# MarioPasc/MGA-YOLO

Measured on AMD Instinct MI355X. Metric: images/s (MaskCBAM fwd+bwd step at P3/P4/P5, YOLOv8n 640x640), higher is better.
Workload: dtype f32; 1 GPU; YOLOv8n+MGA-CBAM P3/P4/P5, 32x640x640 synthetic per GPU, fp32 (BASELINE.json configs[1]); batch_per_gpu=32, global_batch=32, parallelism=dp1, launch=hipGraph replay, 1 graph/step, handoff_kernels=True

## Files before the change

mga_yolo_amd/csrc/api_bwd.hip:

```cpp
#include "host.cuh"
#include "bwd.cuh"
#include "nhwc_bwd.cuh"

static int backward_args(const mgacbam_bwd_level_t& L, NhwcBwdArgs& N, Sig& sig) {
  const bool nhwc = (L.flags & MGACBAM_LAYOUT_NHWC) != 0;
  if (!L.x || !L.gy || !L.ctx || !L.scratch || !L.gx) return fail(MGACBAM_E_NULL, "backward: x / gy / ctx / scratch / gx is NULL");
  if (!L.gw1 || !L.gb1 || !L.gw2 || !L.gb2 || !L.gwsa || !L.gbeta) return fail(MGACBAM_E_NULL, "backward: NULL parameter-gradient pointer");
  if (L.gmask && !L.mask) return fail(MGACBAM_E_NULL, "backward: gmask requested but mask is NULL");
  if (int e = check_level("backward", L)) return e;
  const int VEC = level_vec(nhwc, L.C, L.H, L.W, L.dtype);
  const size_t need = VEC * elem_size(L.dtype);
  if (!aligned_to(L.x, need) || !aligned_to(L.gy, need) || !aligned_to(L.gx, need) || !aligned_to(L.ctx, 16) ||
      !aligned_to(L.scratch, 16) || (L.gmask && !aligned_to(L.gmask, nhwc ? 4 : 16)) || (nhwc && L.mask && !aligned_to(L.mask, 4)))
    return fail(MGACBAM_E_ALIGN, "backward%s: x/gy/gx must be %zu-byte aligned, ctx/scratch 16-byte", nhwc ? " (NHWC)" : "", need);
  const ScratchLayout SL = scratch_layout(L.B, L.C, L.H, L.W, L.p.hidden, L.p.k, nhwc, VEC);
  if (int e = check_ctx_capacity("backward", L)) return e;
  if (int e = check_capacity("backward", "scratch", SL.total, L.scratch_bytes)) return e;
  BwdArgs& A = N.a;
  A.x = L.x; A.mask = L.mask; A.gy = L.gy; A.gx = L.gx; A.gmask = L.gmask;
  A.gw1 = L.gw1; A.gb1 = L.gb1; A.gw2 = L.gw2; A.gb2 = L.gb2; A.gwsa = L.gwsa; A.gbeta = L.gbeta;
  level_setup(L, A);
  A.s = scratch_ptrs(L.scratch, SL);
  A.nconv = A.g.B * conv_tiles(A.t, A.g.H, A.g.W);
  A.nwsa = A.g.B * wsa_tiles(A.t, A.g.H, A.g.W);
  A.npg = params_blocks(A.g);
  A.merged = 0;
  A.vec = VEC;
  sig = Sig{L.dtype, VEC, L.mask != nullptr, L.p.k, L.gmask != nullptr, 0};
  if (nhwc) {
    N.n = nhwc_geo(L.C, L.H, L.W, VEC);
    N.ncb = (L.C + kNhwcFoldC - 1) / kNhwcFoldC;
    A.nt = N.n.nchunk;
    A.ncg = N.ncb;
    A.bflag0 = A.cflag0 = A.mbflag0 = A.mcflag0 = A.wflag0 = A.sflag0 = 0;
    sig.nhwc = 1;
    sig.weight = L.C;
    return 0;
  }
  A.nt = chan_tiles(A.t, A.g.H, A.g.W, VEC);
  A.ncg = 0;
  const SyncLayout S = sync_layout(L.B, L.C, static_cast<size_t>(L.H) * L.W);
  A.bflag0 = static_cast<int>(S.bflag); A.cflag0 = static_cast<int>(S.cflag);
  A.mbflag0 = static_cast<int>(S.mbflag); A.mcflag0 = static_cast<int>(S.mcflag);
  A.wflag0 = static_cast<int>(S.wflag); A.sflag0 = static_cast<int>(S.sflag);
  sig.weight = L.C * A.t.chan_tx;
  sig.proj = (L.flags & MGACBAM_BWD_HAVE_PROJ) && L.gmask != nullptr;
  A.g.proj_h = (sig.proj && L.p.hidden <= MGACBAM_PROJ_MAX_HIDDEN) ? L.p.hidden : 0;
  return 0;
}

template <typename SmemOf>
static size_t group_smem(const Group<BwdArgs>& G, SmemOf smem_of) {
  size_t smem = 0;
  for (int l = 0; l < G.n; ++l) smem = std::max(smem, smem_of(G.lv[l]));
  return smem;
}
static size_t reduce2_smem(const Tune& t) { return (64 + static_cast<size_t>(std::max(kPghLds, kBlock / t.pool_tx))) * sizeof(float); }
static int launch_convT(Group<BwdArgs>& G, int k, hipStream_t st) {
  const size_t smem = group_smem(G, [&](const BwdArgs& a) { return convT_smem(a.t, k); });
  const int grid = fill_starts(G, G.lv, G.n, [](const BwdArgs& a) { return a.nconv; });
  switch (k) {
    case 3: LAUNCH(k_bwd_convT<3>, grid, smem, st, G); break;
    case 5: LAUNCH(k_bwd_convT<5>, grid, smem, st, G); break;
    case 7: LAUNCH(k_bwd_convT<7>, grid, smem, st, G); break;
    default: LAUNCH(k_bwd_convT<0>, grid, smem, st, G); break;
  }
  return launch_status("k_bwd_convT");
}
static int launch_wsa(Group<BwdArgs>& G, int k, hipStream_t st) {
  const size_t smem = group_smem(G, [&](const BwdArgs& a) { return wsa_smem(a.t, k); });
  const int grid = fill_starts(G, G.lv, G.n, [](const BwdArgs& a) { return a.nwsa; });
  switch (k) {
    case 3: LAUNCH(k_bwd_wsa<3>, grid, smem, st, G); break;
    case 5: LAUNCH(k_bwd_wsa<5>, grid, smem, st, G); break;
    case 7: LAUNCH(k_bwd_wsa<7>, grid, smem, st, G); break;
    default: LAUNCH(k_bwd_wsa<0>, grid, smem, st, G); break;
  }
  return launch_status("k_bwd_wsa");
}
static int launch_params(Group<BwdArgs>& G, hipStream_t st) {
  const size_t smem = group_smem(G, [](const BwdArgs& a) { return params_smem(a.g); });
  const int grid = fill_starts(G, G.lv, G.n, [](const BwdArgs& a) { return a.npg; });
  LAUNCH(k_bwd_params, grid, smem, st, G);
  return launch_status("k_bwd_params");
}

static int backward_group(BwdArgs* lv, int n, const Sig& sig, int stages, hipStream_t st) {
  Group<BwdArgs> G;
  G.n = n;
  constexpr int kReduce2MaxCpt = 4;
  const int cpt = group_cpt(lv, n, kReduce2MaxCpt);
  for (int l = 0; l < n; ++l) {
    lv[l].t.pool_cpt = cpt;
    const int cpb = (kBlock / lv[l].t.pool_tx) * cpt;
    lv[l].ncg = (lv[l].g.C + cpb - 1) / cpb;
    G.lv[l] = lv[l];
  }

  bool fold = (stages & MGACBAM_BWD_FOLD) && (stages & MGACBAM_BWD_REDUCE1) && (stages & MGACBAM_BWD_CONVT);
  for (int l = 0; l < n && fold; ++l) {
    const int TP = lv[l].t.chan_tx * sig.vec;
    fold = TP >= kSyncPx && TP >= lv[l].g.W && 8 * (((lv[l].t.conv_th + lv[l].g.k) * lv[l].g.W + TP - 1) / TP + 1) <= 512 &&
           lv[l].nconv <= lv[l].g.B * lv[l].nflag;
  }
  const bool fuse = (stages & MGACBAM_BWD_FUSE) != 0;
  bool merge = fold && fuse && (stages & MGACBAM_BWD_REDUCE2) && (stages & MGACBAM_BWD_WSA) && sig.k == 7 && knobs().bwd_merge;
  for (int l = 0; l < n && merge; ++l) merge = lv[l].nwsa <= lv[l].g.B * lv[l].nflag && lv[l].ncg <= lv[l].g.C && lv[l].nconv % lv[l].g.B == 0;
  if (merge) {
    R12Group R;
    R.g.n = n;
    size_t smem = 0;
    for (int l = 0; l < n; ++l) {
      lv[l].merged = 1; lv[l].bflag0 = lv[l].mbflag0; lv[l].cflag0 = lv[l].mcflag0;
      R.g.lv[l] = lv[l];
      smem = std::max({smem, reduce1_smem(lv[l].g, sig.vec), convT_smem(lv[l].t, sig.k), wsa_smem(lv[l].t, sig.k),
                       reduce2_smem(lv[l].t)});
    }
    int tot = 0;
    for (int p = 0; p < 4; ++p) {
      for (int l = 0; l < n; ++l) {
        R.seg[p][l] = tot;
        tot += p == 0 ? xcd_grid(lv[l].g.B, lv[l].nt) : p == 1 ? pad8(lv[l].nconv) : p == 2 ? pad8(lv[l].nwsa) : sweep_blocks(lv[l], lv[l].t.pool_tx, cpt);
      }
      R.seg[p][n] = tot;
    }
    const int grid = tot;
#define CALL_R12B(CPTV) LAUNCH((k_bwd_r12<TT, VV, CPTV>), grid, smem, st, R)
#define CALL_R12(Tt, Vv) { using TT = Tt; constexpr int VV = Vv; DISPATCH_CPT(cpt, CALL_R12B); }
    DISPATCH_T_VEC(sig.dtype, sig.vec, CALL_R12);
#undef CALL_R12
#undef CALL_R12B
    if (int e = launch_status("k_bwd_r12")) return e;
    for (int l = 0; l < n; ++l) G.lv[l] = lv[l];
  }
  if (fold && !merge) {
    size_t smem = 0;
    for (int l = 0; l < n; ++l) smem = std::max({smem, reduce1_smem(lv[l].g, sig.vec), convT_smem(lv[l].t, sig.k)});
    const int grid = fill_starts(G, lv, n, [&](const BwdArgs& a) { return xcd_grid(a.g.B, a.nt) + pad8(a.nconv); });
#define CALL_R1F(Tt, Vv) if (sig.k == 7) LAUNCH((k_bwd_reduce1_fold<Tt, Vv, 7>), grid, smem, st, G); else LAUNCH((k_bwd_reduce1_fold<Tt, Vv, 0>), grid, smem, st, G)
    DISPATCH_T_VEC(sig.dtype, sig.vec, CALL_R1F);
#undef CALL_R1F
    if (int e = launch_status("k_bwd_reduce1_fold")) return e;
  }
  if ((stages & MGACBAM_BWD_REDUCE1) && !fold) {
    size_t smem = 0;
    for (int l = 0; l < n; ++l) smem = std::max(smem, reduce1_smem(lv[l].g, sig.vec));
    const int grid = fill_starts(G, lv, n, [&](const BwdArgs& a) { return xcd_grid(a.g.B, a.nt); });
#define CALL_R1(Tt, Vv) LAUNCH((k_bwd_reduce1<Tt, Vv>), grid, smem, st, G)
    DISPATCH_T_VEC(sig.dtype, sig.vec, CALL_R1);
#undef CALL_R1
    if (int e = launch_status("k_bwd_reduce1")) return e;
  }
  if ((stages & MGACBAM_BWD_CONVT) && !fold)
    if (int e = launch_convT(G, sig.k, st)) return e;
  const bool fuse_pg = fuse && (stages & MGACBAM_BWD_APPLY) && (stages & MGACBAM_BWD_PARAMGRAD);
  const bool fuse_wsa = fuse && (stages & MGACBAM_BWD_REDUCE2) && (stages & MGACBAM_BWD_WSA) && sig.k == 7;
  if ((stages & MGACBAM_BWD_REDUCE2) && !merge) {
    size_t smem = 0;
    for (int l = 0; l < n; ++l) {
      smem = std::max(smem, reduce2_smem(lv[l].t));
      if (fuse_wsa) smem = std::max(smem, wsa_smem(lv[l].t, sig.k));
    }
    const int grid = fill_starts(G, lv, n, [&](const BwdArgs& a) { return (fuse_wsa ? pad8(a.nwsa) : 0) + sweep_blocks(a, a.t.pool_tx, cpt); });
#define CALL_R22(CPTV) if (fuse_wsa) LAUNCH((k_bwd_reduce2<TT, VV, CPTV, true>), grid, smem, st, G); else LAUNCH((k_bwd_reduce2<TT, VV, CPTV, false>), grid, smem, st, G)
#define CALL_R2(Tt, Vv) { using TT = Tt; constexpr int VV = Vv; DISPATCH_CPT(cpt, CALL_R22); }
    DISPATCH_T_VEC(sig.dtype, sig.vec, CALL_R2);
#undef CALL_R2
#undef CALL_R22
    if (int e = launch_status("k_bwd_reduce2")) return e;
  }
  if ((stages & MGACBAM_BWD_WSA) && !fuse_wsa && !merge)
    if (int e = launch_wsa(G, sig.k, st)) return e;
  if ((stages & MGACBAM_BWD_PARAMGRAD) && !fuse_pg)
    if (int e = launch_params(G, st)) return e;
  if (stages & MGACBAM_BWD_APPLY) {
    size_t smem = 0;
    for (int l = 0; l < n; ++l) {
      smem = std::max(smem, bwd_apply_smem(lv[l].g, sig.vec));
      if (fuse_pg) smem = std::max(smem, params_smem(lv[l].g));
    }
    const int grid = fill_starts(G, lv, n, [&](const BwdArgs& a) { return (fuse_pg ? pad8(a.npg) : 0) + xcd_grid(a.g.B, a.nt); });
#define CALL_AP2(GM) if (fuse_pg) LAUNCH((k_bwd_apply<TT, VV, GM, true>), grid, smem, st, G); else LAUNCH((k_bwd_apply<TT, VV, GM, false>), grid, smem, st, G)
#define CALL_AP(Tt, Vv) { using TT = Tt; constexpr int VV = Vv; if (sig.gmask) { CALL_AP2(true); } else { CALL_AP2(false); } }
    DISPATCH_T_VEC(sig.dtype, sig.vec, CALL_AP);
#undef CALL_AP
#undef CALL_AP2
    if (int e = launch_status("k_bwd_apply")) return e;
  }
  return 0;
}

static int backward_group_nhwc(NhwcBwdArgs* lv, int n, const Sig& sig, int stages, hipStream_t st) {
  Group<NhwcBwdArgs> G;
  Group<BwdArgs> GB;
  G.n = GB.n = n;
  for (int l = 0; l < n; ++l) { G.lv[l] = lv[l]; GB.lv[l] = lv[l].a; }
  auto chunks = [&]() { return fill_starts(G, lv, n, [&](const NhwcBwdArgs& a) { return xcd_grid(a.a.g.B, a.n.nchunk); }); };
  if (stages & MGACBAM_BWD_REDUCE1) {
    size_t smem = 0;
    for (int l = 0; l < n; ++l) smem = std::max(smem, nhwc_reduce1_smem(lv[l].a.g, sig.vec));
    const int grid = chunks();
#define CALL_NR1(Tt, Vv) LAUNCH((k_bwd_reduce1_nhwc<Tt, Vv>), grid, smem, st, G)
    DISPATCH_T_VEC8(sig.dtype, sig.vec, CALL_NR1);
#undef CALL_NR1
    if (int e = launch_status("k_bwd_reduce1_nhwc")) return e;
  }
  if (stages & MGACBAM_BWD_CONVT)
    if (int e = launch_convT(GB, sig.k, st)) return e;
  if (stages & MGACBAM_BWD_REDUCE2) {
    size_t smem = 0;
    for (int l = 0; l < n; ++l) smem = std::max(smem, nhwc_reduce2_smem(lv[l].a.g));
    const int grid = chunks();
#define CALL_NR2(Tt, Vv) LAUNCH((k_bwd_reduce2_nhwc<Tt, Vv>), grid, smem, st, G)
    DISPATCH_T_VEC8(sig.dtype, sig.vec, CALL_NR2);
#undef CALL_NR2
    if (int e = launch_status("k_bwd_reduce2_nhwc")) return e;
    const int fgrid = fill_starts(G, lv, n, [&](const NhwcBwdArgs& a) { return a.a.g.B * a.ncb; });
    LAUNCH(k_bwd_fold_nhwc, fgrid, 0, st, G);
    if (int e = launch_status("k_bwd_fold_nhwc")) return e;
  }
  if (stages & MGACBAM_BWD_WSA)
    if (int e = launch_wsa(GB, sig.k, st)) return e;
  if (stages & MGACBAM_BWD_PARAMGRAD)
    if (int e = launch_params(GB, st)) return e;
  if (stages & MGACBAM_BWD_APPLY) {
    size_t smem = 0;
    for (int l = 0; l < n; ++l) smem = std::max(smem, nhwc_bwd_apply_smem(lv[l].a.g));
    const int grid = fill_starts(G, lv, n, [&](const NhwcBwdArgs& a) { return xcd_grid(a.a.g.B, a.n.ntile); });
#define CALL_NAP(Tt, Vv) if (sig.gmask) LAUNCH((k_bwd_apply_nhwc<Tt, Vv, true>), grid, smem, st, G); else LAUNCH((k_bwd_apply_nhwc<Tt, Vv, false>), grid, smem, st, G)
    DISPATCH_T_VEC8(sig.dtype, sig.vec, CALL_NAP);
#undef CALL_NAP
// ... 30 lines not shown
```

mga_yolo_amd/csrc/args.cuh:

```cuda
#pragma once
#include <stddef.h>
#include <stdint.h>

namespace mgacbam {

struct Geo {
  int B, C, H, W, HW;
  int hidden, k;
  int use_sigmoid;
  float thr, eps;
  int proj_h;
};
constexpr int kProjMax = 4;
constexpr int kGateR = 16;
constexpr int kSyncPx = 16;

struct CtxPtrs {
  float* S; float* use; float* den;
  float* avg; float* mx; float* mavg;
  int* valid; int* amax;
  float* h_avg; float* h_mx; float* ca;
  float* planes; int* cidx; float* sa;
  float* proj;
  int* sync;
};

struct ParamPtrs { const float* w1; const float* b1; const float* w2; const float* b2; const float* wsa; const float* beta; };

struct Tune {
  int pool_tx;
  int pool_cpt;
  int chan_tx;
  int conv_twq;
  int conv_th;
  int wsa_th;
  int apply_rows;
  int gate_rows;
  int gate_tx;
  int gate_span;
};

struct FwdArgs {
  const void* x; const float* mask; void* y;
  CtxPtrs c; ParamPtrs p; Geo g; Tune t;
  int nflag;
  int fused;
  unsigned spin_limit;
  int fault;
  long long* trace;
};

struct ScratchPtrs {
  float* A_part;
  float* gpre;
  float* gplanes;
  float* gwsa_part;
  float* gz;
  float* gbq;
  float* gh_avg;
  float* gh_mx;
  float* pgh;
};

struct BwdArgs {
  const void* x; const float* mask; const void* gy; void* gx; float* gmask;
  float* gw1; float* gb1; float* gw2; float* gb2; float* gwsa; float* gbeta;
  CtxPtrs c; ParamPtrs p; ScratchPtrs s; Geo g; Tune t;
  int nt;
  int nconv;
  int nwsa;
  int npg;
  int ncg;
  int nflag;
  int bflag0;
  int cflag0;
  int wflag0;
  int sflag0;
  int mbflag0, mcflag0;
  int merged;
  unsigned spin_limit;
  int vec;
  long long* trace;
};

struct NhwcGeo {
  int cs, lcs;
  int ng;
  int ch;
  int ntile;
  int rp;
  int nchunk;
};
constexpr int kNhwcMaxChunks = 64;
constexpr int kNhwcFoldC = 64;

static inline size_t align16(size_t v) { return (v + 15) & ~size_t(15); }

constexpr int kGroupMax = 4;
template <typename Args>
struct Group {
  int n;
  int start[kGroupMax + 1];
  Args lv[kGroupMax];
};

}
```

mga_yolo_amd/csrc/bwd.cuh:

```cuda
#pragma once
#include "args.cuh"
#include "common.cuh"
#include "tile.cuh"

namespace mgacbam {

constexpr int kPghLds = 2048;

template <typename T, int VEC, bool FOLD = false>
__device__ __forceinline__ void bwd_reduce1_body(const BwdArgs& A, const int bid, float* smem) {
  const Geo& g = A.g;
  const int tid = threadIdx.x;
  const int TX = A.t.chan_tx, lt = ilog2(TX);
  const int tx = tid & (TX - 1), ty = tid >> lt, TY = kBlock >> lt;
  const int nv = g.HW / VEC;
  const int ntile = A.nt;
  int b, tile;
  if (!xcd_sample_part(bid, g.B, ntile, b, tile)) return;
  const int i = tile * TX + tx;
  const bool active = i < nv;
  const int ii = active ? i : nv - 1;
  const size_t base = static_cast<size_t>(b) * g.C * g.HW + static_cast<size_t>(ii) * VEC;
  const T* xp = static_cast<const T*>(A.x) + base;
  const T* gp = static_cast<const T*>(A.gy) + base;
  const float a = softplusf_(*A.p.beta);
  float* s_ca = smem;
  float* s_aq = smem + g.C;
  float* sm = s_aq + 2 * g.C;
  for (int c = tid; c < g.C; c += kBlock) s_ca[c] = A.c.ca[static_cast<size_t>(b) * g.C + c];

  float sav[VEC];
  load_vec<float, VEC>(A.c.sa + static_cast<size_t>(b) * g.HW + static_cast<size_t>(ii) * VEC, sav);
  const float live = active ? 1.f : 0.f;
  float accp[VEC];
#pragma unroll
  for (int e = 0; e < VEC; ++e) accp[e] = 0.f;
  __syncthreads();

#pragma unroll 4
  for (int c = ty; c < g.C; c += TY) {
    float xv[VEC], gv[VEC];
    load_vec<T, VEC>(xp + static_cast<size_t>(c) * g.HW, xv);
    load_vec<T, VEC>(gp + static_cast<size_t>(c) * g.HW, gv);
    const float cac = s_ca[c];
    float pa = 0.f, pq = 0.f;
#pragma unroll
    for (int e = 0; e < VEC; ++e) {
      const float p = xv[e] * gv[e] * live;
      accp[e] += cac * p;
      pa += p * sav[e];
      pq += p * (cac * sav[e] - 1.f);
    }
    pa = wave_group_sum(pa, TX);
    pq = wave_group_sum(pq, TX);
    if (tx == 0) { s_aq[c] = pa; s_aq[g.C + c] = pq; }
  }
#pragma unroll
  for (int e = 0; e < VEC; ++e) sm[tid * VEC + e] = accp[e];
  __syncthreads();
  float* part = A.s.A_part + (static_cast<size_t>(b) * ntile + tile) * 2 * g.C;
  if (FOLD && A.merged) { for (int c = tid; c < 2 * g.C; c += kBlock) st_agent(part + c, s_aq[c]); }
  else { for (int c = tid; c < 2 * g.C; c += kBlock) part[c] = s_aq[c]; }
  if (ty == 0 && active) {
    for (int r = 1; r < TY; ++r) {
      const int o = (r * TX + tx) * VEC;
#pragma unroll
      for (int e = 0; e < VEC; ++e) accp[e] += sm[o + e];
    }
    float gpre[VEC];
#pragma unroll
    for (int e = 0; e < VEC; ++e) gpre[e] = a * accp[e] * sav[e] * (1.f - sav[e]);
    float* gq = A.s.gpre + static_cast<size_t>(b) * g.HW + static_cast<size_t>(i) * VEC;
    if (FOLD) {
#pragma unroll
      for (int e = 0; e < VEC; ++e) st_agent(gq + e, gpre[e]);
    } else {
      store_vec<float, VEC>(gq, gpre);
    }
  }
  if (FOLD) handoff_publish(A.c.sync + A.bflag0 + static_cast<size_t>(b) * A.nflag + tile);
}

template <typename T, int VEC>
__global__ __launch_bounds__(kBlock) void k_bwd_reduce1(const Group<BwdArgs> G) {
  extern __shared__ __align__(16) float smem[];
  int local;
  const int l = find_level(G, blockIdx.x, local);
  bwd_reduce1_body<T, VEC>(G.lv[l], local, smem);
}

template <int K, bool COH>
__device__ __forceinline__ void bwd_convT_body(const BwdArgs& A, const int local, float* smem) {
  const Geo& g = A.g;
  const int k = K ? K : g.k;
  const ConvTile c = conv_tile(g, A.t, k, local, A.t.conv_th);
  const int tid = threadIdx.x;
  float* wts = smem;
  float* tg = smem + ((3 * k * k + 3) & ~3);
  for (int i = tid; i < 3 * k * k; i += kBlock) wts[i] = A.p.wsa[i];
  const float* gpre = A.s.gpre + static_cast<size_t>(c.b) * g.HW;
  bool bad = false;
  if (COH) {
    int* own = A.c.sync + A.cflag0 + local;
    const int gen = static_cast<int>(static_cast<unsigned>(ld_agent(own)) + 1u);
    const int TP = A.t.chan_tx * A.vec;
    const int ra = max(c.y0 - c.pad, 0), rb = min(c.y0 + c.TH - 1 + c.pad, g.H - 1);
    bad = handoff_wait(A.c.sync + A.bflag0 + static_cast<size_t>(c.b) * A.nflag, (ra * g.W) / TP, ((rb + 1) * g.W - 1) / TP, gen,
                       A.c.sync + static_cast<size_t>(g.B) * A.nflag, A.spin_limit);
    if (tid == 0 && !A.merged) __hip_atomic_fetch_add(own, 1, __ATOMIC_RELAXED, __HIP_MEMORY_SCOPE_AGENT);
  }
  stage_window<8>(tg, 1, c.PH, c.PW, c.y0 - c.pad, c.x0 - c.pad, g, [&](int, int off) { return COH ? ld_agent(gpre + off) : gpre[off]; });
  __syncthreads();
  const int TWQ = A.t.conv_twq;
  const int py = tid / TWQ, q = tid - py * TWQ;
  constexpr int KK = K ? K : 1;
  const bool publish = COH && A.merged;
  if (py >= c.TH && !publish) return;
  float acc[3][4];
#pragma unroll
  for (int p = 0; p < 3; ++p)
#pragma unroll
    for (int e = 0; e < 4; ++e) acc[p][e] = 0.f;
  if (py >= c.TH) {
  } else if (K) {
#pragma unroll 1
    for (int i = 0; i < KK; ++i) {
      const float* row = tg + (py + i) * c.PW + q * 4;
      float r[4 + KK - 1];
#pragma unroll
      for (int t = 0; t < 4 + KK - 1; ++t) r[t] = row[t];
#pragma unroll
      for (int p = 0; p < 3; ++p) {
        const float* wr = wts + (p * KK + (KK - 1 - i)) * KK;
#pragma unroll
        for (int j = 0; j < KK; ++j) {
          const float wv = wr[KK - 1 - j];
#pragma unroll
          for (int e = 0; e < 4; ++e) acc[p][e] += wv * r[e + j];
        }
      }
    }
  } else {
    for (int i = 0; i < k; ++i) {
      const float* row = tg + (py + i) * c.PW + q * 4;
      for (int j = 0; j < k; ++j) {
#pragma unroll
        for (int p = 0; p < 3; ++p) {
          const float wv = wts[(p * k + (k - 1 - i)) * k + (k - 1 - j)];
#pragma unroll
          for (int e = 0; e < 4; ++e) acc[p][e] += wv * row[e + j];
        }
      }
    }
  }
  const int yg = c.y0 + py;
  if (py < c.TH && yg < g.H) {
#pragma unroll
    for (int e = 0; e < 4; ++e) {
      const int xg = c.x0 + q * 4 + e;
      if (xg < g.W) {
#pragma unroll
        for (int p = 0; p < 3; ++p) {
          float* dst = A.s.gplanes + (static_cast<size_t>(c.b) * 3 + p) * g.HW + yg * g.W + xg;
          const float v = bad ? __builtin_nanf("") : acc[p][e];
          if (publish) st_agent(dst, v); else *dst = v;
        }
      }
    }
  }
  if (publish) handoff_publish(A.c.sync + A.cflag0 + local);
}

template <int K>
__global__ __launch_bounds__(kBlock) void k_bwd_convT(const Group<BwdArgs> G) {
  extern __shared__ __align__(16) float smem[];
  int local;
  const int lvl = find_level(G, blockIdx.x, local);
  bwd_convT_body<K, false>(G.lv[lvl], local, smem);
}

template <typename T, int VEC, int K>
__global__ __launch_bounds__(kBlock) void k_bwd_reduce1_fold(const Group<BwdArgs> G) {
  extern __shared__ __align__(16) float smem[];
  int local;
  const int l = find_level(G, blockIdx.x, local);
  const BwdArgs& A = G.lv[l];
  const int tiles = ((A.g.B + 7) / 8) * 8 * A.nt;
  if (local >= tiles) {
    if (local - tiles < A.nconv) bwd_convT_body<K, true>(A, local - tiles, smem);
    return;
  }
  bwd_reduce1_body<T, VEC, true>(A, local, smem);
}

template <int K, bool COH = false>
__device__ __forceinline__ void bwd_wsa_body(const BwdArgs& A, const int local, float* smem) {
  const Geo& g = A.g;
  const int k = K ? K : g.k;
  const ConvTile c = conv_tile(g, A.t, k, local, A.t.wsa_th);
  const int tid = threadIdx.x;
  const int plane_elems = c.PH * c.PW;
  float* tg = smem;
  float* tp = tg + plane_elems;
  float* accs = tp + 3 * plane_elems;
  const float* gpre = A.s.gpre + static_cast<size_t>(c.b) * g.HW;
  const float* pl = A.c.planes + static_cast<size_t>(c.b) * 3 * g.HW;
  bool bad = false;
  if (COH) {
    int* own = A.c.sync + A.wflag0 + local;
    const int gen = static_cast<int>(static_cast<unsigned>(ld_agent(own)) + 1u);
    const int TP = A.t.chan_tx * A.vec;
    const int ra = max(c.y0 - c.pad, 0), rb = min(c.y0 + c.TH - 1 + c.pad, g.H - 1);
    bad = handoff_wait(A.c.sync + A.bflag0 + static_cast<size_t>(c.b) * A.nflag, (ra * g.W) / TP, ((rb + 1) * g.W - 1) / TP, gen,
                       A.c.sync + static_cast<size_t>(g.B) * A.nflag, A.spin_limit);
    if (tid == 0) __hip_atomic_fetch_add(own, 1, __ATOMIC_RELAXED, __HIP_MEMORY_SCOPE_AGENT);
  }
  stage_window<8>(tg, 4, c.PH, c.PW, c.y0 - c.pad, c.x0 - c.pad, g,
                   [&](int p, int off) { return p == 0 ? (COH ? ld_agent(gpre + off) : gpre[off]) : pl[static_cast<size_t>(p - 1) * g.HW + off]; });
  __syncthreads();
  constexpr int KK = K ? K : 1;
  const int nout = 3 * k * k;
  if (K) {
    const int nitems = 3 * KK * c.TH;
    for (int item = tid; item < nitems; item += kBlock) {
      const int pi = item / c.TH, r = item - pi * c.TH;
      const int p = pi / KK, i = pi - p * KK;
      const float* prow = tp + p * plane_elems + (r + i) * c.PW;
      const float* grow = tg + (r + c.pad) * c.PW + c.pad;
      float acc[KK];
#pragma unroll
      for (int j = 0; j < KK; ++j) acc[j] = 0.f;
      float w[KK + 3];
#pragma unroll
      for (int t = 0; t < KK - 1; ++t) w[t] = prow[t];
      for (int x = 0; x < c.TW; x += 4) {
        float gq[4];
#pragma unroll
        for (int e = 0; e < 4; ++e) { gq[e] = grow[x + e]; w[KK - 1 + e] = prow[x + KK - 1 + e]; }
#pragma unroll
        for (int e = 0; e < 4; ++e)
#pragma unroll
          for (int j = 0; j < KK; ++j) acc[j] += gq[e] * w[e + j];
#pragma unroll
        for (int t = 0; t < KK - 1; ++t) w[t] = w[t + 4];
      }
#pragma unroll
      for (int j = 0; j < KK; ++j) accs[item * KK + j] = acc[j];
    }
    __syncthreads();
    for (int o = tid; o < nout; o += kBlock) {
      const int pi = o / KK, j = o - pi * KK;
      float sum = 0.f;
      for (int r = 0; r < c.TH; ++r) sum += accs[(pi * c.TH + r) * KK + j];
      if (COH && bad) sum = __builtin_nanf("");
      A.s.gwsa_part[static_cast<size_t>(o) * A.nwsa + local] = sum;
    }
  } else {
    for (int o = tid; o < nout; o += kBlock) {
      const int p = o / (k * k), r = o - p * k * k;
      const int i = r / k, j = r - i * k;
      const float* pp = tp + p * plane_elems + i * c.PW + j;
      const float* gg = tg + c.pad * c.PW + c.pad;
      float sum = 0.f;
      for (int yy = 0; yy < c.TH; ++yy)
        for (int xx = 0; xx < c.TW; ++xx) sum += gg[yy * c.PW + xx] * pp[yy * c.PW + xx];
      A.s.gwsa_part[static_cast<size_t>(o) * A.nwsa + local] = sum;
    }
  }
}

template <int K>
__global__ __launch_bounds__(kBlock) void k_bwd_wsa(const Group<BwdArgs> G) {
  extern __shared__ __align__(16) float smem[];
  int local;
  const int lvl = find_level(G, blockIdx.x, local);
// ... 95 lines not shown
    const float* part = A.s.A_part + static_cast<size_t>(b) * A.nt * 2 * g.C + cj[j];
    float As = 0.f, Qs = 0.f;
    if (COH) { for (int t = tx; t < A.nt; t += TX) { As += ld_agent(part + static_cast<size_t>(t) * 2 * g.C); Qs += ld_agent(part + static_cast<size_t>(t) * 2 * g.C + g.C); } }
    else { for (int t = tx; t < A.nt; t += TX) { As += part[static_cast<size_t>(t) * 2 * g.C]; Qs += part[static_cast<size_t>(t) * 2 * g.C + g.C]; } }
    sums[j] = acc[j]; sums[CPT + j] = As; sums[2 * CPT + j] = Qs;
  }
  row_sum<3 * CPT>(sums, TX, tid, red);
  float gzv[CPT];
#pragma unroll
  for (int j = 0; j < CPT; ++j) gzv[j] = 0.f;
  if (tx == 0) {
    const float a = softplusf_(*A.p.beta);
#pragma unroll
    for (int j = 0; j < CPT; ++j) {
      const int c = c0 + j;
      if (c < g.C) {
        const size_t o = static_cast<size_t>(b) * g.C + c;
        const float As = sums[CPT + j], Qs = sums[2 * CPT + j];
        const float ca = A.c.ca[o];
        const float gca = a * As + sums[j];
        gzv[j] = (COH && bad) ? __builtin_nanf("") : gca * ca * (1.f - ca);
        A.s.gz[o] = gzv[j];
        A.s.gbq[o] = Qs;
      }
    }
  }
  const int h = g.hidden;
  float* s_pg = red + 64;
  const int hc = min(h, max(1, kPghLds / TY));
  for (int h0 = 0; h0 < h; h0 += hc) {
    const int hn = min(hc, h - h0);
    if (h0) __syncthreads();
    if (tx == 0) {
      for (int jh = 0; jh < hn; ++jh) {
        float p = 0.f;
#pragma unroll
        for (int j = 0; j < CPT; ++j) p += A.p.w2[static_cast<size_t>(cj[j]) * h + h0 + jh] * gzv[j];
        s_pg[ty * hc + jh] = p;
      }
    }
    __syncthreads();
    for (int jh = tid; jh < hn; jh += kBlock) {
      float p = 0.f;
      for (int r = 0; r < TY; ++r) p += s_pg[r * hc + jh];
      A.s.pgh[(static_cast<size_t>(b) * ncg + cg) * h + h0 + jh] = p;
    }
  }
}

template <typename T, int VEC, int CPT, bool ROLES>
__global__ __launch_bounds__(kBlock) void k_bwd_reduce2(const Group<BwdArgs> G) {
  extern __shared__ __align__(16) float smem[];
  int local;
  const int l = find_level(G, blockIdx.x, local);
  const BwdArgs& A = G.lv[l];
  if (ROLES) {
    const int npad = (A.nwsa + 7) & ~7;
    if (local < npad) {
      if (local < A.nwsa) {
        TRACE_MARK(A.trace, blockIdx.x, 0);
        bwd_wsa_body<7>(A, local, smem);
#ifdef MGACBAM_TRACE
        asm volatile("s_waitcnt vmcnt(0)" ::: "memory");
        __syncthreads();
        TRACE_MARK(A.trace, blockIdx.x, 5);
#endif
      }
      return;
    }
    local -= npad;
  }
  TRACE_MARK(A.trace, blockIdx.x, 0);
  bwd_reduce2_body<T, VEC, CPT>(A, local, smem);
#ifdef MGACBAM_TRACE
  asm volatile("s_waitcnt vmcnt(0)" ::: "memory");
  TRACE_MARK(A.trace, blockIdx.x, 10);
#endif
}

struct R12Group {
  Group<BwdArgs> g;
  int seg[4][kGroupMax + 1];
};
template <typename T, int VEC, int CPT>
__global__ __launch_bounds__(kBlock) void k_bwd_r12(const R12Group R) {
  extern __shared__ __align__(16) float smem[];
  const int bid = blockIdx.x;
  int p = 0;
#pragma unroll
  for (int q = 1; q < 4; ++q)
    if (bid >= R.seg[q][0]) p = q;
  int l = 0;
#pragma unroll
  for (int i = 1; i < kGroupMax; ++i)
    if (i < R.g.n && bid >= R.seg[p][i]) l = i;
  const int local = bid - R.seg[p][l];
  const BwdArgs& A = R.g.lv[l];
#ifdef MGACBAM_TRACE
  TRACE_MARK(A.trace, blockIdx.x, 0);
  if (A.trace && threadIdx.x == 0) A.trace[static_cast<size_t>(blockIdx.x) * 16 + 14] = p + 1;
#endif
  if (p == 0) bwd_reduce1_body<T, VEC, true>(A, local, smem);
  else if (p == 1) { if (local < A.nconv) bwd_convT_body<7, true>(A, local, smem); }
  else if (p == 2) { if (local < A.nwsa) bwd_wsa_body<7, true>(A, local, smem); }
  else bwd_reduce2_body<T, VEC, CPT, true>(A, local, smem);
#ifdef MGACBAM_TRACE
  asm volatile("s_waitcnt vmcnt(0)" ::: "memory");
  __syncthreads();
  TRACE_MARK(A.trace, blockIdx.x, 10);
#endif
}

__device__ __forceinline__ void bwd_params_body(const BwdArgs& A, const int local, float* sm, float* red) {
  const Geo& g = A.g;
  const int C = g.C, h = g.hidden, B = g.B, kk3 = 3 * g.k * g.k;
  const int nb2 = (C + kBlock - 1) / kBlock, nb_wsa = (kk3 + 3) / 4;
  const int tid = threadIdx.x, wave = tid >> 6, lane = tid & 63;
  if (local < h) {
    const int j = local;
    float* s_ga = sm; float* s_gm = sm + B; float* s_hs = sm + 2 * B;
    float* s_part = sm + 3 * B;
#pragma unroll 2
    for (int b = wave; b < B; b += kBlock / kWave) {
      const float* gz = A.s.gz + static_cast<size_t>(b) * C;
      float d = 0.f;
#pragma unroll 4
      for (int c = lane; c < C; c += kWave) d += A.p.w2[static_cast<size_t>(c) * h + j] * gz[c];
      d = wave_group_sum(d, kWave);
      if (lane == 0) {
        const float ha = A.c.h_avg[b * h + j], hm = A.c.h_mx[b * h + j];
        const float ga = ha > 0.f ? d : 0.f, gm = hm > 0.f ? d : 0.f;
        s_ga[b] = ga; s_gm[b] = gm; s_hs[b] = ha + hm;
        A.s.gh_avg[b * h + j] = ga;
        A.s.gh_mx[b * h + j] = gm;
      }
    }
    __syncthreads();
    const int cp = (C >= kBlock) ? kBlock : C;
    const int ng = kBlock / cp;
    const int cl = tid % cp, bg = tid / cp;
    for (int c0 = 0; c0 < C; c0 += cp) {
      const int c = c0 + cl;
      float w1 = 0.f, w2 = 0.f;
      if (c < C && bg < ng) {
#pragma unroll 4
        for (int b = bg; b < B; b += ng) {
          const size_t o = static_cast<size_t>(b) * C + c;
          w1 += s_ga[b] * A.c.avg[o] + s_gm[b] * A.c.mx[o];
          w2 += A.s.gz[o] * s_hs[b];
        }
      }
      if (ng > 1) {
        __syncthreads();
        s_part[tid] = w1; s_part[kBlock + tid] = w2;
        __syncthreads();
        if (bg == 0 && c < C) {
          for (int q = 1; q < ng; ++q) { w1 += s_part[q * cp + cl]; w2 += s_part[kBlock + q * cp + cl]; }
        }
      }
      if (bg == 0 && c < C) {
        A.gw1[static_cast<size_t>(j) * C + c] = w1;
        A.gw2[static_cast<size_t>(c) * h + j] = w2;
      }
    }
    if (tid == 0) {
      float acc = 0.f;
      for (int b = 0; b < B; ++b) acc += s_ga[b] + s_gm[b];
      A.gb1[j] = acc;
    }
    return;
  }
  if (local < h + nb2) {
    const int c = (local - h) * kBlock + tid;
    if (c >= C) return;
    float acc = 0.f;
#pragma unroll 8
    for (int b = 0; b < B; ++b) acc += A.s.gz[static_cast<size_t>(b) * C + c];
    A.gb2[c] = 2.f * acc;
    return;
  }
  if (local < h + nb2 + nb_wsa) {
    const int o = (local - h - nb2) * 4 + wave;
    if (o >= kk3) return;
    const float* part = A.s.gwsa_part + static_cast<size_t>(o) * A.nwsa;
    float acc = 0.f;
// ... 250 lines not shown
```

mga_yolo_amd/csrc/host.cuh:

```cuda
#pragma once
#include "../../include/mgacbam.h"

#include <hip/hip_runtime.h>
#include <stdarg.h>
#include <stdio.h>
#include <stdlib.h>
#include <string.h>

#include <algorithm>
#include <atomic>
#include <map>
#include <mutex>
#include <utility>

#include "args.cuh"
#include "common.cuh"

using namespace mgacbam;

inline thread_local char g_err[512] = "";
static int fail(int code, const char* fmt, ...) {
  va_list ap;
  va_start(ap, fmt);
  vsnprintf(g_err, sizeof(g_err), fmt, ap);
// ... 315 lines not shown
template <typename Level>
static int check_level(const char* what, const Level& L) {
  if (int e = check_params(L.p)) return e;
  if (int e = check_shape(L.B, L.C, L.H, L.W, L.p.hidden, L.p.k)) return e;
  if (L.dtype < MGACBAM_F32 || L.dtype > MGACBAM_BF16) return fail(MGACBAM_E_DTYPE, "%s: dtype %d", what, L.dtype);
  return 0;
}
template <typename Level>
static int check_ctx_capacity(const char* what, const Level& L) {
  mgacbam_ctx_layout_t CL;
  ctx_layout(L.B, L.C, L.H, L.W, L.p.hidden, &CL);
  return check_capacity(what, "ctx", static_cast<size_t>(CL.total), L.ctx_bytes);
}
template <typename Level, typename Args>
static void level_setup(const Level& L, Args& A) {
  A.c = ctx_ptrs(const_cast<void*>(static_cast<const void*>(L.ctx)), L.B, L.C, L.H, L.W, L.p.hidden);
  A.p = make_params(L.p);
  A.g = make_geo(L.B, L.C, L.H, L.W, L.p);
  A.t = choose_tune(L.B, L.C, L.H, L.W, L.p.k);
  A.nflag = static_cast<int>(sync_layout(L.B, L.C, static_cast<size_t>(L.H) * L.W).nflag);
  const Knobs kn = knobs();
  A.trace = kn.trace; A.spin_limit = kn.spin_limit;
}

struct Sig {
  int dtype, vec, has_mask, k, gmask, proj;
  int lf32 = 0;
  int nhwc = 0;
  int cvec = 0;
  int gvec = 0;
  int weight = 0;
  bool operator==(const Sig& o) const {
    return dtype == o.dtype && vec == o.vec && has_mask == o.has_mask && k == o.k && gmask == o.gmask && proj == o.proj && gvec == o.gvec && lf32 == o.lf32 && nhwc == o.nhwc && cvec == o.cvec;
  }
};

template <typename Args>
static int group_cpt(const Args* lv, int n, int max_cpt = 2) {
  const int forced = knobs().pool_cpt;
  if (forced == 1 || forced == 2 || forced == 4) return forced;
  for (int cpt = max_cpt; cpt > 1; cpt /= 2) {
    long long blocks = 0;
    for (int l = 0; l < n; ++l) {
      const int tx = lv[l].t.pool_tx;
      const int cpb = (kBlock / tx) * cpt;
      blocks += static_cast<long long>(lv[l].g.B) * ((lv[l].g.C + cpb - 1) / cpb);
    }
    if (blocks >= 1536) return cpt;
  }
  return 1;
}
static int xcd_grid(int B, int parts) { return ((B + 7) / 8) * 8 * parts; }
static int pad8(int n) { return (n + 7) & ~7; }
template <typename Args>
static int sweep_blocks(const Args& a, int tx, int cpt) {
  const int cpb = (kBlock / tx) * cpt;
  return xcd_grid(a.g.B, (a.g.C + cpb - 1) / cpb);
}
static size_t convT_smem(const Tune& t, int k) {
  return (((3 * k * k + 3) & ~3) + static_cast<size_t>(t.conv_th + k - 1) * (t.conv_twq * 4 + k - 1)) * sizeof(float);
}
static size_t wsa_smem(const Tune& t, int k) {
  return (4 * static_cast<size_t>(t.wsa_th + k - 1) * (t.conv_twq * 4 + k - 1) + static_cast<size_t>(3 * k * t.wsa_th) * k) * sizeof(float);
}
static size_t params_smem(const Geo& g) { return (3 * static_cast<size_t>(g.B) + 2 * kBlock) * sizeof(float); }
static int params_blocks(const Geo& g) { return g.hidden + (g.C + kBlock - 1) / kBlock + (3 * g.k * g.k + 3) / 4 + 1; }
static size_t chan_smem(const Geo& g, int vec, bool proj) {
  return (3 * static_cast<size_t>(g.C) + 2 * g.hidden + (proj ? static_cast<size_t>(g.C) * kProjMax : 0) + 4 * kBlock * vec) * sizeof(float);
}
static size_t apply_smem(const Geo& g, const Tune& t, int vec) {
  return (((3 * g.k * g.k + 3) & ~3) + 3 * static_cast<size_t>(t.apply_rows) * (g.W + g.k - 1) + t.chan_tx * vec + g.C) * sizeof(float);
}
static size_t gate_smem(const Geo& g, const Tune& t, int vec) {
  const size_t head = (g.C + 3) & ~3;
  const size_t role = 3 * static_cast<size_t>(g.C) + 2 * g.hidden;
  const size_t conv = ((3 * g.k * g.k + 3) & ~3) + 3 * static_cast<size_t>(t.gate_rows) * (g.W + g.k - 1) + static_cast<size_t>(t.gate_tx) * vec;
  return std::max(role, head + std::max(conv, static_cast<size_t>(3) * kBlock * vec)) * sizeof(float);
}
static int gate_tiles(const Tune& t, int H, int W, int vec) {
  const int nv = H * W / vec;
  return (nv + t.gate_tx - 1) / t.gate_tx;
}
static size_t bwd_apply_smem(const Geo& g, int vec) { return (5 * static_cast<size_t>(g.C) + 2 * g.hidden + kBlock * vec) * sizeof(float); }
static size_t reduce1_smem(const Geo& g, int vec) { return (3 * static_cast<size_t>(g.C) + kBlock * vec) * sizeof(float); }
static size_t mlp_smem(const Geo& g) { return (3 * static_cast<size_t>(g.C) + 2 * g.hidden) * sizeof(float); }
static size_t nhwc_pool_smem(const Geo& g) { return 4 * static_cast<size_t>(g.C) * sizeof(float); }
static size_t nhwc_chan_smem(const Geo& g) { return static_cast<size_t>(g.C) * sizeof(float); }
static size_t nhwc_apply_smem(const Geo& g, const Tune& t, const NhwcGeo& n) {
  return (((3 * g.k * g.k + 3) & ~3) + 3 * static_cast<size_t>(t.apply_rows) * (g.W + g.k - 1) + n.ch + g.C) * sizeof(float);
}
static size_t nhwc_reduce1_smem(const Geo& g, int vec) {
  return (3 * ((static_cast<size_t>(g.C) + 3) & ~static_cast<size_t>(3)) + 2 * kBlock * vec) * sizeof(float);
}
static size_t nhwc_reduce2_smem(const Geo& g) { return static_cast<size_t>(g.C) * sizeof(float); }
static size_t nhwc_bwd_apply_smem(const Geo& g) { return (5 * static_cast<size_t>(g.C) + 2 * g.hidden) * sizeof(float); }

template <typename Args, typename Fn>
static int fill_starts(Group<Args>& G, const Args* lv, int n, Fn blocks_of) {
  int tot = 0;
  for (int l = 0; l < n; ++l) { G.start[l] = tot; tot += blocks_of(lv[l]); }
  G.start[n] = tot;
  return tot;
}

template <typename Args, typename Run>
static int for_each_group(Args* args, const Sig* sigs, int n, Run run) {
  bool done[MGACBAM_MAX_LEVELS] = {false};
  for (int l = 0; l < n; ++l) {
    if (done[l]) continue;
    int idx[kGroupMax], m = 0;
    for (int j = l; j < n && m < kGroupMax; ++j)
      if (!done[j] && sigs[j] == sigs[l]) { idx[m++] = j; done[j] = true; }
    std::stable_sort(idx, idx + m, [&](int a, int b) { return sigs[a].weight > sigs[b].weight; });
    Args grp[kGroupMax];
    for (int j = 0; j < m; ++j) grp[j] = args[idx[j]];
    if (int e = run(grp, m, sigs[l])) return e;
  }
  return 0;
}
```

Baseline: 162,300 images/s.

## Compute mask projection inside backward reduce1 when forward did not save it

When the forward pass has not stored the W1·x projection needed for the mask gradient, the backward reduce1 kernel now computes it. It stages W1 transposed in shared memory and accumulates per-hidden-unit dot products while it already streams x across channels, then reduces across the thread rows and writes the projection to the context buffer. This lets the later mask-gradient path use the cheaper precomputed-projection route instead of recomputing, at the cost of more registers, more LDS and extra syncs in reduce1.

```diff
diff --git a/mga_yolo_amd/csrc/api_bwd.hip b/mga_yolo_amd/csrc/api_bwd.hip
--- a/mga_yolo_amd/csrc/api_bwd.hip
+++ b/mga_yolo_amd/csrc/api_bwd.hip
@@ -25,6 +25,7 @@
   A.nwsa = A.g.B * wsa_tiles(A.t, A.g.H, A.g.W);
   A.npg = params_blocks(A.g);
   A.merged = 0;
+  A.make_proj = 0;
   A.vec = VEC;
   sig = Sig{L.dtype, VEC, L.mask != nullptr, L.p.k, L.gmask != nullptr, 0};
   if (nhwc) {
@@ -44,8 +45,11 @@
   A.mbflag0 = static_cast<int>(S.mbflag); A.mcflag0 = static_cast<int>(S.mcflag);
   A.wflag0 = static_cast<int>(S.wflag); A.sflag0 = static_cast<int>(S.sflag);
   sig.weight = L.C * A.t.chan_tx;
-  sig.proj = (L.flags & MGACBAM_BWD_HAVE_PROJ) && L.gmask != nullptr;
-  A.g.proj_h = (sig.proj && L.p.hidden <= MGACBAM_PROJ_MAX_HIDDEN) ? L.p.hidden : 0;
+  const bool have = (L.flags & MGACBAM_BWD_HAVE_PROJ) != 0;
+  const bool make = !have && L.dtype == MGACBAM_F32 && reduce1_smem(A.g, VEC, true) <= 64 * 1024;
+  sig.proj = L.gmask != nullptr;
+  A.g.proj_h = (L.gmask && L.p.hidden <= MGACBAM_PROJ_MAX_HIDDEN && (have || make)) ? L.p.hidden : 0;
+  A.make_proj = A.g.proj_h > 0 && make;
   return 0;
 }
 
@@ -103,6 +107,8 @@
     fold = TP >= kSyncPx && TP >= lv[l].g.W && 8 * (((lv[l].t.conv_th + lv[l].g.k) * lv[l].g.W + TP - 1) / TP + 1) <= 512 &&
            lv[l].nconv <= lv[l].g.B * lv[l].nflag;
   }
+  bool mkproj = false;
+  for (int l = 0; l < n; ++l) mkproj = mkproj || lv[l].make_proj;
   const bool fuse = (stages & MGACBAM_BWD_FUSE) != 0;
   bool merge = fold && fuse && (stages & MGACBAM_BWD_REDUCE2) && (stages & MGACBAM_BWD_WSA) && sig.k == 7 && knobs().bwd_merge;
   for (int l = 0; l < n && merge; ++l) merge = lv[l].nwsa <= lv[l].g.B * lv[l].nflag && lv[l].ncg <= lv[l].g.C && lv[l].nconv % lv[l].g.B == 0;
@@ -113,7 +119,7 @@
     for (int l = 0; l < n; ++l) {
       lv[l].merged = 1; lv[l].bflag0 = lv[l].mbflag0; lv[l].cflag0 = lv[l].mcflag0;
       R.g.lv[l] = lv[l];
-      smem = std::max({smem, reduce1_smem(lv[l].g, sig.vec), convT_smem(lv[l].t, sig.k), wsa_smem(lv[l].t, sig.k),
+      smem = std::max({smem, reduce1_smem(lv[l].g, sig.vec, lv[l].make_proj), convT_smem(lv[l].t, sig.k), wsa_smem(lv[l].t, sig.k),
                        reduce2_smem(lv[l].t)});
     }
     int tot = 0;
@@ -125,7 +131,7 @@
       R.seg[p][n] = tot;
     }
     const int grid = tot;
-#define CALL_R12B(CPTV) LAUNCH((k_bwd_r12<TT, VV, CPTV>), grid, smem, st, R)
+#define CALL_R12B(CPTV) if (mkproj) LAUNCH((k_bwd_r12<TT, VV, CPTV, true>), grid, smem, st, R); else LAUNCH((k_bwd_r12<TT, VV, CPTV, false>), grid, smem, st, R)
 #define CALL_R12(Tt, Vv) { using TT = Tt; constexpr int VV = Vv; DISPATCH_CPT(cpt, CALL_R12B); }
     DISPATCH_T_VEC(sig.dtype, sig.vec, CALL_R12);
 #undef CALL_R12
@@ -135,18 +141,20 @@
   }
   if (fold && !merge) {
     size_t smem = 0;
-    for (int l = 0; l < n; ++l) smem = std::max({smem, reduce1_smem(lv[l].g, sig.vec), convT_smem(lv[l].t, sig.k)});
+    for (int l = 0; l < n; ++l) smem = std::max({smem, reduce1_smem(lv[l].g, sig.vec, lv[l].make_proj), convT_smem(lv[l].t, sig.k)});
     const int grid = fill_starts(G, lv, n, [&](const BwdArgs& a) { return xcd_grid(a.g.B, a.nt) + pad8(a.nconv); });
-#define CALL_R1F(Tt, Vv) if (sig.k == 7) LAUNCH((k_bwd_reduce1_fold<Tt, Vv, 7>), grid, smem, st, G); else LAUNCH((k_bwd_reduce1_fold<Tt, Vv, 0>), grid, smem, st, G)
+#define CALL_R1F2(Tt, Vv, PJ) if (sig.k == 7) LAUNCH((k_bwd_reduce1_fold<Tt, Vv, 7, PJ>), grid, smem, st, G); else LAUNCH((k_bwd_reduce1_fold<Tt, Vv, 0, PJ>), grid, smem, st, G)
+#define CALL_R1F(Tt, Vv) if (mkproj) { CALL_R1F2(Tt, Vv, true); } else { CALL_R1F2(Tt, Vv, false); }
     DISPATCH_T_VEC(sig.dtype, sig.vec, CALL_R1F);
 #undef CALL_R1F
+#undef CALL_R1F2
     if (int e = launch_status("k_bwd_reduce1_fold")) return e;
   }
   if ((stages & MGACBAM_BWD_REDUCE1) && !fold) {
     size_t smem = 0;
-    for (int l = 0; l < n; ++l) smem = std::max(smem, reduce1_smem(lv[l].g, sig.vec));
+    for (int l = 0; l < n; ++l) smem = std::max(smem, reduce1_smem(lv[l].g, sig.vec, lv[l].make_proj));
     const int grid = fill_starts(G, lv, n, [&](const BwdArgs& a) { return xcd_grid(a.g.B, a.nt); });
-#define CALL_R1(Tt, Vv) LAUNCH((k_bwd_reduce1<Tt, Vv>), grid, smem, st, G)
+#define CALL_R1(Tt, Vv) if (mkproj) LAUNCH((k_bwd_reduce1<Tt, Vv, true>), grid, smem, st, G); else LAUNCH((k_bwd_reduce1<Tt, Vv, false>), grid, smem, st, G)
     DISPATCH_T_VEC(sig.dtype, sig.vec, CALL_R1);
 #undef CALL_R1
     if (int e = launch_status("k_bwd_reduce1")) return e;
diff --git a/mga_yolo_amd/csrc/args.cuh b/mga_yolo_amd/csrc/args.cuh
--- a/mga_yolo_amd/csrc/args.cuh
+++ b/mga_yolo_amd/csrc/args.cuh
@@ -77,6 +77,7 @@
   int wflag0;
   int sflag0;
   int mbflag0, mcflag0;
+  int make_proj;
   int merged;
   unsigned spin_limit;
   int vec;
diff --git a/mga_yolo_amd/csrc/bwd.cuh b/mga_yolo_amd/csrc/bwd.cuh
--- a/mga_yolo_amd/csrc/bwd.cuh
+++ b/mga_yolo_amd/csrc/bwd.cuh
@@ -7,8 +7,10 @@
 
 constexpr int kPghLds = 2048;
 
-template <typename T, int VEC, bool FOLD = false>
+template <typename T, int VEC, bool FOLD = false, bool PROJ = false>
 __device__ __forceinline__ void bwd_reduce1_body(const BwdArgs& A, const int bid, float* smem) {
+  constexpr int HP = kProjMax;
+  static_assert(HP % 4 == 0, "the W1 rows of a channel are read as float4");
   const Geo& g = A.g;
   const int tid = threadIdx.x;
   const int TX = A.t.chan_tx, lt = ilog2(TX);
@@ -26,8 +28,18 @@
   const float a = softplusf_(*A.p.beta);
   float* s_ca = smem;
   float* s_aq = smem + g.C;
-  float* sm = s_aq + 2 * g.C;
+  const bool proj = PROJ && A.make_proj;
+  float* s_w1t = smem + ((3 * g.C + 3) & ~3);
+  float* sm = proj ? s_w1t + g.C * HP : s_aq + 2 * g.C;
   for (int c = tid; c < g.C; c += kBlock) s_ca[c] = A.c.ca[static_cast<size_t>(b) * g.C + c];
+  if (PROJ) {
+    if (proj) {
+      for (int idx = tid; idx < g.C * HP; idx += kBlock) {
+        const int c = idx / HP, j = idx - c * HP;
+        s_w1t[idx] = j < g.proj_h ? A.p.w1[static_cast<size_t>(j) * g.C + c] : 0.f;
+      }
+    }
+  }
 
   float sav[VEC];
   load_vec<float, VEC>(A.c.sa + static_cast<size_t>(b) * g.HW + static_cast<size_t>(ii) * VEC, sav);
@@ -35,6 +47,11 @@
   float accp[VEC];
 #pragma unroll
   for (int e = 0; e < VEC; ++e) accp[e] = 0.f;
+  float accP[PROJ ? HP : 1][VEC];
+#pragma unroll
+  for (int j = 0; j < (PROJ ? HP : 1); ++j)
+#pragma unroll
+    for (int e = 0; e < VEC; ++e) accP[j][e] = 0.f;
   __syncthreads();
 
 #pragma unroll 4
@@ -43,6 +60,20 @@
     load_vec<T, VEC>(xp + static_cast<size_t>(c) * g.HW, xv);
     load_vec<T, VEC>(gp + static_cast<size_t>(c) * g.HW, gv);
     const float cac = s_ca[c];
+    if (PROJ) {
+      if (proj) {
+        float w[HP];
+#pragma unroll
+        for (int q4 = 0; q4 < HP / 4; ++q4) {
+          const float4 wv = *reinterpret_cast<const float4*>(s_w1t + c * HP + 4 * q4);
+          w[4 * q4] = wv.x; w[4 * q4 + 1] = wv.y; w[4 * q4 + 2] = wv.z; w[4 * q4 + 3] = wv.w;
+        }
+#pragma unroll
+        for (int j = 0; j < HP; ++j)
+#pragma unroll
+          for (int e = 0; e < VEC; ++e) accP[j][e] += w[j] * xv[e];
+      }
+    }
     float pa = 0.f, pq = 0.f;
 #pragma unroll
     for (int e = 0; e < VEC; ++e) {
@@ -79,14 +110,43 @@
     }
   }
   if (FOLD) handoff_publish(A.c.sync + A.bflag0 + static_cast<size_t>(b) * A.nflag + tile);
-}
-
-template <typename T, int VEC>
+  if (PROJ) {
+    if (proj) {
+#pragma unroll
+      for (int half = 0; half < HP / 4; ++half) {
+        if (half * 4 >= g.proj_h) break;
+        if (!FOLD || half) __syncthreads();
+#pragma unroll
+        for (int jj = 0; jj < 4; ++jj)
+#pragma unroll
+          for (int e = 0; e < VEC; ++e) sm[(jj * kBlock + tid) * VEC + e] = accP[half * 4 + jj][e];
+        __syncthreads();
+        if (ty == 0 && active) {
+#pragma unroll
+          for (int jj = 0; jj < 4; ++jj) {
+            const int j = half * 4 + jj;
+            if (j < g.proj_h) {
+              float pv[VEC];
+#pragma unroll
+              for (int e = 0; e < VEC; ++e) pv[e] = accP[j][e];
+              for (int r = 1; r < TY; ++r)
+#pragma unroll
+                for (int e = 0; e < VEC; ++e) pv[e] += sm[(jj * kBlock + r * TX + tx) * VEC + e];
+              store_vec<float, VEC>(A.c.proj + (static_cast<size_t>(b) * g.proj_h + j) * g.HW + static_cast<size_t>(i) * VEC, pv);
+            }
+          }
+        }
+      }
+    }
+  }
+}
+
+template <typename T, int VEC, bool PROJ>
 __global__ __launch_bounds__(kBlock) void k_bwd_reduce1(const Group<BwdArgs> G) {
   extern __shared__ __align__(16) float smem[];
   int local;
   const int l = find_level(G, blockIdx.x, local);
-  bwd_reduce1_body<T, VEC>(G.lv[l], local, smem);
+  bwd_reduce1_body<T, VEC, false, PROJ>(G.lv[l], local, smem);
 }
 
 template <int K, bool COH>
@@ -179,7 +239,7 @@
   bwd_convT_body<K, false>(G.lv[lvl], local, smem);
 }
 
-template <typename T, int VEC, int K>
+template <typename T, int VEC, int K, bool PROJ>
 __global__ __launch_bounds__(kBlock) void k_bwd_reduce1_fold(const Group<BwdArgs> G) {
   extern __shared__ __align__(16) float smem[];
   int local;
@@ -190,7 +250,7 @@
     if (local - tiles < A.nconv) bwd_convT_body<K, true>(A, local - tiles, smem);
     return;
   }
-  bwd_reduce1_body<T, VEC, true>(A, local, smem);
+  bwd_reduce1_body<T, VEC, true, PROJ>(A, local, smem);
 }
 
 template <int K, bool COH = false>
@@ -452,7 +512,7 @@
   Group<BwdArgs> g;
   int seg[4][kGroupMax + 1];
 };
-template <typename T, int VEC, int CPT>
+template <typename T, int VEC, int CPT, bool PROJ>
 __global__ __launch_bounds__(kBlock) void k_bwd_r12(const R12Group R) {
   extern __shared__ __align__(16) float smem[];
   const int bid = blockIdx.x;
@@ -470,7 +530,7 @@
   TRACE_MARK(A.trace, blockIdx.x, 0);
   if (A.trace && threadIdx.x == 0) A.trace[static_cast<size_t>(blockIdx.x) * 16 + 14] = p + 1;
 #endif
-  if (p == 0) bwd_reduce1_body<T, VEC, true>(A, local, smem);
+  if (p == 0) bwd_reduce1_body<T, VEC, true, PROJ>(A, local, smem);
   else if (p == 1) { if (local < A.nconv) bwd_convT_body<7, true>(A, local, smem); }
   else if (p == 2) { if (local < A.nwsa) bwd_wsa_body<7, true>(A, local, smem); }
   else bwd_reduce2_body<T, VEC, CPT, true>(A, local, smem);
diff --git a/mga_yolo_amd/csrc/host.cuh b/mga_yolo_amd/csrc/host.cuh
--- a/mga_yolo_amd/csrc/host.cuh
+++ b/mga_yolo_amd/csrc/host.cuh
@@ -421,7 +421,10 @@
   return (nv + t.gate_tx - 1) / t.gate_tx;
 }
 static size_t bwd_apply_smem(const Geo& g, int vec) { return (5 * static_cast<size_t>(g.C) + 2 * g.hidden + kBlock * vec) * sizeof(float); }
-static size_t reduce1_smem(const Geo& g, int vec) { return (3 * static_cast<size_t>(g.C) + kBlock * vec) * sizeof(float); }
+static size_t reduce1_smem(const Geo& g, int vec, bool proj) {
+  if (!proj) return (3 * static_cast<size_t>(g.C) + kBlock * vec) * sizeof(float);
+  return (((3 * static_cast<size_t>(g.C) + 3) & ~static_cast<size_t>(3)) + static_cast<size_t>(g.C) * kProjMax + 4 * kBlock * vec) * sizeof(float);
+}
 static size_t mlp_smem(const Geo& g) { return (3 * static_cast<size_t>(g.C) + 2 * g.hidden) * sizeof(float); }
 static size_t nhwc_pool_smem(const Geo& g) { return 4 * static_cast<size_t>(g.C) * sizeof(float); }
 static size_t nhwc_chan_smem(const Geo& g) { return static_cast<size_t>(g.C) * sizeof(float); }
```

Measured after the change: 165,500 images/s, median of 6. 1.02x the previous value.
